# yeyupiaoling/VoiceprintRecognition-PaddlePaddle

Hardware: NVIDIA H100
Metric: utterances/sec ECAPA-TDNN Fbank80 3s embed extract (higher is better)
Workload: dtype bf16x3 (split-bf16 operands, fp32 accumulate; fp32-grade)

## Files before the change

voiceprintrecognition-paddlepaddle_b200/csrc/asp_fused.cu:

```cuda
#include <stdio.h>
#include <string.h>

#include "common.h"
#include "ptx.cuh"

namespace ppv {

constexpr int AF_NT = 64;
constexpr int AF_A_TILE = 128 * 64 * 2;
constexpr int AF_B_TILE = AF_NT * 64 * 2;
constexpr int AF_X_TILE = AF_NT * 128 * 2;
constexpr int AF_STAGES = 2;
constexpr float LOG2E = 1.4426950408889634f;

template <int NSPLIT>
__global__ void __launch_bounds__(384, 1) asp_fused_kernel(const __grid_constant__ AspFusedParams p) {
    constexpr int NP = (NSPLIT == 3) ? 2 : 1;
    extern __shared__ uint8_t smem_raw[];
    const uint32_t smem_base = (smem_u32(smem_raw) + 1023u) & ~1023u;
    uint8_t* smem_gen = smem_raw + (smem_base - smem_u32(smem_raw));
    const int ksteps = p.K / 64;
    const int a_bytes = ksteps * NP * AF_A_TILE;
    const int b_bytes = ksteps * NP * AF_B_TILE;
    const int stage_bytes = b_bytes + 2 * AF_X_TILE;
    const uint32_t a_base = smem_base;
    const uint32_t s_base = smem_base + a_bytes;
    const uint32_t bar_base = s_base + AF_STAGES * stage_bytes;
    const uint32_t a_full = bar_base, a_empty = bar_base + 8;
    auto b_full = [&](int s) { return bar_base + 16u + 8u * s; };
    auto b_empty = [&](int s) { return bar_base + 32u + 8u * s; };

    const int warp = threadIdx.x >> 5, lane = threadIdx.x & 31;
    if (warp == 0 && lane == 0) {
        prefetch_tmap(&p.mapW);
        prefetch_tmap(&p.mapAtt);
        prefetch_tmap(&p.mapX);
    }
    if (warp == 1 && lane == 0) {
        mbar_init(a_full, 1);
        mbar_init(a_empty, 256);
        for (int s = 0; s < AF_STAGES; ++s) {
            mbar_init(b_full(s), 1);
            mbar_init(b_empty(s), 256);
        }
        fence_mbar_init();
    }
    __syncthreads();
    griddep_launch_dependents();
    griddep_wait();

    const int slabs = p.C / 128;
    const int items = slabs * p.B;
    const int ntiles = (p.T + AF_NT - 1) / AF_NT;

    if (warp == 0) {
        int stage = 0;
        uint32_t phase = 0, a_phase = 0;
        int cur_slab = -1;
        for (int item = blockIdx.x; item < items; item += gridDim.x) {
            const int b = item / slabs, slab = item - b * slabs;
            if (slab != cur_slab) {
                mbar_wait(a_empty, a_phase ^ 1u);
                if (lane == 0) {
                    mbar_arrive_expect_tx(a_full, a_bytes);
                    for (int ks = 0; ks < ksteps; ++ks)
                        for (int pl = 0; pl < NP; ++pl)
                            tma_load_3d(a_base + (ks * NP + pl) * AF_A_TILE, &p.mapW, a_full, ks * 64, slab * 128, pl);
                }
                __syncwarp();
                a_phase ^= 1u;
                cur_slab = slab;
            }
            {
                const int nitem = item + gridDim.x;
                if (nitem < items && lane < 2 * ntiles) {
                    const int nb = nitem / slabs, nslab = nitem - nb * slabs;
                    tma_prefetch_l2_3d(&p.mapX, nslab * 128, nb * p.Tp + p.P + (lane >> 1) * AF_NT, lane & 1);
                }
                __syncwarp();
            }
            const int row0 = b * p.Tp + p.P;
            for (int ft = 0; ft < ntiles; ++ft) {
                mbar_wait(b_empty(stage), phase ^ 1u);
                if (lane == 0) {
                    const uint32_t sb = s_base + stage * stage_bytes;
                    mbar_arrive_expect_tx(b_full(stage), stage_bytes);
                    for (int ks = 0; ks < ksteps; ++ks)
                        for (int pl = 0; pl < NP; ++pl)
                            tma_load_3d(sb + (ks * NP + pl) * AF_B_TILE, &p.mapAtt, b_full(stage), ks * 64, row0 + ft * AF_NT, pl);
                    for (int pl = 0; pl < 2; ++pl)
                        tma_load_3d(sb + b_bytes + pl * AF_X_TILE, &p.mapX, b_full(stage), slab * 128, row0 + ft * AF_NT, pl);
                }
                __syncwarp();
                if (++stage == AF_STAGES) {
                    stage = 0;
                    phase ^= 1u;
                }
            }
        }
    } else if (warp >= 4) {
        const int g = (warp - 4) >> 2, t = threadIdx.x & 127, w = t >> 5, l = t & 31;
        const int cl0 = 64 * g + 16 * w + (l >> 2);
        float acc[AF_NT / 2];
#pragma unroll
        for (int i = 0; i < AF_NT / 2; ++i) acc[i] = 0.f;
        int stage = 0;
        uint32_t phase = 0, a_phase = 0;
        int cur_slab = -1;
        for (int item = blockIdx.x; item < items; item += gridDim.x) {
            const int b = item / slabs, slab = item - b * slabs;
            if (slab != cur_slab) {
                mbar_wait(a_full, a_phase);
                a_phase ^= 1u;
                cur_slab = slab;
            }
            const int nitem = item + gridDim.x;
            const bool last_of_slab = (nitem >= items) || (nitem % slabs != slab);
            float gm[2], m[2], S0[2], S1[2], S2[2];
#pragma unroll
            for (int rr = 0; rr < 2; ++rr) {
                const int64_t goff = int64_t(b) * p.gstat.ld + slab * 128 + cl0 + 8 * rr;
                gm[rr] = __bfloat162float(p.gstat.hi()[goff]) + __bfloat162float(p.gstat.lo()[goff]);
                m[rr] = -INFINITY;
                S0[rr] = S1[rr] = S2[rr] = 0.f;
            }
            const int Tb = p.nvalid ? max(1, min(p.T, p.nvalid[b])) : p.T;
            for (int ft = 0; ft < ntiles; ++ft) {
                mbar_wait(b_full(stage), phase);
                const uint32_t sb = s_base + stage * stage_bytes;
                wgmma_fence_acc(acc);
                wgmma_fence();
                for (int ks = 0; ks < ksteps; ++ks) {
                    const uint64_t a_hi = make_sw128_kmajor_desc(a_base + (ks * NP) * AF_A_TILE + g * 64 * 128);
                    const uint64_t b_hi = make_sw128_kmajor_desc(sb + (ks * NP) * AF_B_TILE);
#pragma unroll
                    for (int k = 0; k < 4; ++k) wgmma_bf16<AF_NT>(acc, a_hi + 2 * k, b_hi + 2 * k, (ks > 0 || k > 0) ? 1u : 0u);
                    if (NSPLIT == 3) {
                        const uint64_t a_lo = make_sw128_kmajor_desc(a_base + (ks * NP + 1) * AF_A_TILE + g * 64 * 128);
                        const uint64_t b_lo = make_sw128_kmajor_desc(sb + (ks * NP + 1) * AF_B_TILE);
#pragma unroll
                        for (int k = 0; k < 4; ++k) wgmma_bf16<AF_NT>(acc, a_lo + 2 * k, b_hi + 2 * k, 1u);
#pragma unroll
                        for (int k = 0; k < 4; ++k) wgmma_bf16<AF_NT>(acc, a_hi + 2 * k, b_lo + 2 * k, 1u);
                    }
                }
                wgmma_commit();
                wgmma_wait<0>();
                wgmma_fence_acc(acc);
                if (ft == ntiles - 1 && last_of_slab) mbar_arrive(a_empty);
                const __nv_bfloat16* xs_hi = reinterpret_cast<const __nv_bfloat16*>(smem_gen + (sb - smem_base) + b_bytes);
                const __nv_bfloat16* xs_lo = xs_hi + AF_X_TILE / 2;
                const int f0 = ft * AF_NT;
#pragma unroll
                for (int rr = 0; rr < 2; ++rr) {
                    float cm = -INFINITY;
#pragma unroll
                    for (int i = 0; i < AF_NT / 8; ++i)
#pragma unroll
                        for (int e = 0; e < 2; ++e)
                            if (f0 + 8 * i + 2 * (l & 3) + e < Tb) cm = fmaxf(cm, acc[4 * i + 2 * rr + e]);
                    if (cm > m[rr]) {
                        const float r = exp2f((m[rr] - cm) * LOG2E);
                        S0[rr] *= r;
                        S1[rr] *= r;
                        S2[rr] *= r;
                        m[rr] = cm;
                    }
                    const float ms = m[rr] * LOG2E;
                    const int cl = cl0 + 8 * rr;
#pragma unroll
                    for (int i = 0; i < AF_NT / 8; ++i)
#pragma unroll
                        for (int e = 0; e < 2; ++e) {
                            const int fl = 8 * i + 2 * (l & 3) + e;
                            if (f0 + fl < Tb) {
                                const int o = fl * 128 + cl;
                                const float xv = __bfloat162float(xs_hi[o]) + __bfloat162float(xs_lo[o]);
                                const float ev = exp2f(fmaf(acc[4 * i + 2 * rr + e], LOG2E, -ms));
                                const float d = xv - gm[rr];
                                const float ed = ev * d;
                                S0[rr] += ev;
                                S1[rr] += ed;
                                S2[rr] = fmaf(ed, d, S2[rr]);
                            }
                        }
                }
                mbar_arrive(b_empty(stage));
                if (++stage == AF_STAGES) {
                    stage = 0;
                    phase ^= 1u;
                }
            }
#pragma unroll
            for (int rr = 0; rr < 2; ++rr) {
#pragma unroll
                for (int off = 1; off <= 2; off <<= 1) {
                    const float om = __shfl_xor_sync(0xffffffffu, m[rr], off), o0 = __shfl_xor_sync(0xffffffffu, S0[rr], off),
                                o1 = __shfl_xor_sync(0xffffffffu, S1[rr], off), o2 = __shfl_xor_sync(0xffffffffu, S2[rr], off);
                    const float mm = fmaxf(m[rr], om);
                    const float ra = S0[rr] > 0.f ? exp2f((m[rr] - mm) * LOG2E) : 0.f, rb = o0 > 0.f ? exp2f((om - mm) * LOG2E) : 0.f;
                    S0[rr] = S0[rr] * ra + o0 * rb;
                    S1[rr] = S1[rr] * ra + o1 * rb;
                    S2[rr] = S2[rr] * ra + o2 * rb;
                    m[rr] = mm;
                }
            }
            if ((l & 3) != 0) continue;
            const int C = p.C;
#pragma unroll
            for (int rr = 0; rr < 2; ++rr) {
                const int c = slab * 128 + cl0 + 8 * rr;
                const float inv = 1.f / S0[rr];
                const float dm = S1[rr] * inv;
                const float mean = gm[rr] + dm;
                const float sd = sqrtf(fmaxf(S2[rr] * inv - dm * dm, p.eps));
                if (p.out_raw) {
                    p.out_raw[int64_t(b) * 2 * C + c] = mean;
                    p.out_raw[int64_t(b) * 2 * C + C + c] = sd;
                }
                __nv_bfloat16 h, lo;
                split_bf16(fmaf(mean, p.bn_scale[c], p.bn_shift[c]), h, lo);
                p.out.hi()[int64_t(b) * p.out.ld + c] = h;
                p.out.lo()[int64_t(b) * p.out.ld + c] = lo;
                split_bf16(fmaf(sd, p.bn_scale[C + c], p.bn_shift[C + c]), h, lo);
                p.out.hi()[int64_t(b) * p.out.ld + C + c] = h;
                p.out.lo()[int64_t(b) * p.out.ld + C + c] = lo;
            }
        }
    }
}

int asp_fused_build(AspFusedParams* p, const Planes& W, const Planes& att, const Planes& x, const Planes& gstat, const float* bn_scale,
                    const float* bn_shift, const Planes& out, float* out_raw, int B, int T, int P, int Tp, int C, int K, float eps) {
    PPV_REQUIRE(C % 128 == 0 && K % 64 == 0 && K <= 128, "asp_fused: C % 128 == 0 and K in {64,128} required");
    memset(p, 0, sizeof(*p));
    PPV_REQUIRE(x.ld == C, "asp_fused: x row length must equal C");
    int rc = encode_planes_map(&p->mapW, W, 128);
    if (rc) return rc;
    rc = encode_planes_map(&p->mapAtt, att, AF_NT);
    if (rc) return rc;
    rc = encode_planes_map_ex(&p->mapX, x, 128, AF_NT, 0);
    if (rc) return rc;
    p->x = x;
    p->gstat = gstat;
    p->bn_scale = bn_scale;
    p->bn_shift = bn_shift;
    p->out = out;
    p->out_raw = out_raw;
    p->B = B;
    p->T = T;
    p->P = P;
    p->Tp = Tp;
    p->C = C;
    p->K = K;
    p->eps = eps;
    p->nvalid = nullptr;
    return PPV_OK;
}

int asp_fused_launch(const AspFusedParams& p, int precision, int num_sms, cudaStream_t st) {
    const bool x3 = precision == PPV_PREC_BF16X3;
    const int ksteps = p.K / 64, np = x3 ? 2 : 1;
    const int smem = 1024 + ksteps * np * AF_A_TILE + AF_STAGES * (ksteps * np * AF_B_TILE + 2 * AF_X_TILE) + 96 + 128 * 16 + 64;
    static bool attr3 = false, attr1 = false;
    bool& attr = x3 ? attr3 : attr1;
    if (!attr) {
        if (x3)
            PPV_CUDA_OK(cudaFuncSetAttribute(asp_fused_kernel<3>, cudaFuncAttributeMaxDynamicSharedMemorySize, 227 * 1024));
        else
            PPV_CUDA_OK(cudaFuncSetAttribute(asp_fused_kernel<1>, cudaFuncAttributeMaxDynamicSharedMemorySize, 227 * 1024));
        attr = true;
    }
    const int items = (p.C / 128) * p.B;
    const int grid = std::min(items, num_sms);
    if (x3)
        PPV_PDL_OK(launch_pdl(asp_fused_kernel<3>, dim3(grid), dim3(384), size_t(smem), st, p), "asp_fused_kernel");
    else
        PPV_PDL_OK(launch_pdl(asp_fused_kernel<1>, dim3(grid), dim3(384), size_t(smem), st, p), "asp_fused_kernel");
    return PPV_OK;
}

}
```

voiceprintrecognition-paddlepaddle_b200/csrc/ptx.cuh:

```cuda
#pragma once
#include <cuda.h>
#include <cuda_bf16.h>
#include <cuda_runtime.h>
#include <stdint.h>
#include <stdio.h>

namespace ppv {

__device__ __forceinline__ uint32_t smem_u32(const void* p) {
    return static_cast<uint32_t>(__cvta_generic_to_shared(p));
}

__device__ __forceinline__ bool elect_one() {
    uint32_t pred = 0;
    asm volatile(
        "{\n\t.reg .pred P;\n\t"
        "elect.sync _|P, 0xffffffff;\n\t"
        "selp.u32 %0, 1, 0, P;\n\t}\n"
        : "=r"(pred));
    return pred != 0;
}

__device__ __forceinline__ void mbar_init(uint32_t bar, uint32_t count) {
    asm volatile("mbarrier.init.shared::cta.b64 [%0], %1;" ::"r"(bar), "r"(count) : "memory");
}
__device__ __forceinline__ void fence_mbar_init() {
    asm volatile("fence.mbarrier_init.release.cluster;" ::: "memory");
}
__device__ __forceinline__ void mbar_arrive(uint32_t bar) {
    asm volatile("mbarrier.arrive.shared::cta.b64 _, [%0];" ::"r"(bar) : "memory");
}
__device__ __forceinline__ void mbar_arrive_expect_tx(uint32_t bar, uint32_t bytes) {
    asm volatile("mbarrier.arrive.expect_tx.shared::cta.b64 _, [%0], %1;" ::"r"(bar), "r"(bytes) : "memory");
}
__device__ __forceinline__ uint32_t mbar_try_wait(uint32_t bar, uint32_t parity) {
    uint32_t done;
    asm volatile(
        "{\n\t.reg .pred P;\n\t"
        "mbarrier.try_wait.parity.shared::cta.b64 P, [%1], %2;\n\t"
        "selp.u32 %0, 1, 0, P;\n\t}\n"
        : "=r"(done)
        : "r"(bar), "r"(parity)
        : "memory");
    return done;
}
__device__ __forceinline__ uint64_t global_timer_ns() {
    uint64_t t;
    asm volatile("mov.u64 %0, %%globaltimer;" : "=l"(t));
    return t;
}
__device__ __forceinline__ void mbar_wait(uint32_t bar, uint32_t parity) {
    if (mbar_try_wait(bar, parity)) return;
    const uint64_t t0 = global_timer_ns();
    uint32_t spins = 0;
    while (!mbar_try_wait(bar, parity)) {
        if ((++spins & 0x3ff) == 0 && global_timer_ns() - t0 > 4000000000ull) __trap();
    }
}

template <int N>
__device__ __forceinline__ void setmaxnreg_dec() { asm volatile("setmaxnreg.dec.sync.aligned.u32 %0;" ::"n"(N)); }
template <int N>
__device__ __forceinline__ void setmaxnreg_inc() { asm volatile("setmaxnreg.inc.sync.aligned.u32 %0;" ::"n"(N)); }

__device__ __forceinline__ void prefetch_tmap(const CUtensorMap* m) {
    asm volatile("prefetch.tensormap [%0];" ::"l"(reinterpret_cast<uint64_t>(m)) : "memory");
}
__device__ __forceinline__ void tma_load_3d(uint32_t smem_dst, const CUtensorMap* m, uint32_t bar, int c0, int c1,
                                            int c2) {
    asm volatile(
        "cp.async.bulk.tensor.3d.shared::cluster.global.mbarrier::complete_tx::bytes"
        " [%0], [%1, {%3, %4, %5}], [%2];"
        :
        : "r"(smem_dst), "l"(reinterpret_cast<uint64_t>(m)), "r"(bar), "r"(c0), "r"(c1), "r"(c2)
        : "memory");
}
__device__ __forceinline__ void tma_prefetch_l2_3d(const CUtensorMap* m, int c0, int c1, int c2) {
    asm volatile("cp.async.bulk.prefetch.tensor.3d.L2.global.tile [%0, {%1, %2, %3}];"
                 :
                 : "l"(reinterpret_cast<uint64_t>(m)), "r"(c0), "r"(c1), "r"(c2)
                 : "memory");
}
__device__ __forceinline__ void tma_store_3d(const CUtensorMap* m, uint32_t smem_src, int c0, int c1, int c2) {
    asm volatile("cp.async.bulk.tensor.3d.global.shared::cta.bulk_group [%0, {%2, %3, %4}], [%1];"
                 :
                 : "l"(reinterpret_cast<uint64_t>(m)), "r"(smem_src), "r"(c0), "r"(c1), "r"(c2)
                 : "memory");
}
__device__ __forceinline__ void bulk_commit_group() { asm volatile("cp.async.bulk.commit_group;" ::: "memory"); }
__device__ __forceinline__ void bulk_wait_read0() { asm volatile("cp.async.bulk.wait_group.read 0;" ::: "memory"); }
__device__ __forceinline__ void bulk_wait_all() { asm volatile("cp.async.bulk.wait_group 0;" ::: "memory"); }
__device__ __forceinline__ void fence_proxy_async_smem() { asm volatile("fence.proxy.async.shared::cta;" ::: "memory"); }
__device__ __forceinline__ void bulk_load_1d(uint32_t smem_dst, const void* gsrc, uint32_t bytes, uint32_t bar) {
    asm volatile(
        "cp.async.bulk.shared::cluster.global.mbarrier::complete_tx::bytes [%0], [%1], %2, [%3];"
        :
        : "r"(smem_dst), "l"(reinterpret_cast<uint64_t>(gsrc)), "r"(bytes), "r"(bar)
        : "memory");
}

__device__ __forceinline__ void wgmma_fence() { asm volatile("wgmma.fence.sync.aligned;" ::: "memory"); }
__device__ __forceinline__ void wgmma_commit() { asm volatile("wgmma.commit_group.sync.aligned;" ::: "memory"); }
template <int N>
__device__ __forceinline__ void wgmma_wait() { asm volatile("wgmma.wait_group.sync.aligned %0;" ::"n"(N) : "memory"); }
template <int R>
__device__ __forceinline__ void wgmma_fence_acc(float (&d)[R]) {
#pragma unroll
    for (int i = 0; i < R; ++i) asm volatile("" : "+f"(d[i])::"memory");
}
__device__ __forceinline__ void wgmma_m64n32k16(float (&d)[16], uint64_t desc_a, uint64_t desc_b, uint32_t scale_d) {
    asm volatile(
        "{\n\t.reg .pred p;\n\t"
        "setp.ne.b32 p, %18, 0;\n\t"
        "wgmma.mma_async.sync.aligned.m64n32k16.f32.bf16.bf16 "
        "{%0, %1, %2, %3, %4, %5, %6, %7, %8, %9, %10, %11, %12, %13, %14, %15}, "
        "%16, %17, p, 1, 1, 0, 0;\n\t}\n"
        : "+f"(d[0]), "+f"(d[1]), "+f"(d[2]), "+f"(d[3]), "+f"(d[4]), "+f"(d[5]), "+f"(d[6]), "+f"(d[7]), "+f"(d[8]), "+f"(d[9]), "+f"(d[10]), "+f"(d[11]), "+f"(d[12]), "+f"(d[13]), "+f"(d[14]), "+f"(d[15])
        : "l"(desc_a), "l"(desc_b), "r"(scale_d));
}
__device__ __forceinline__ void wgmma_m64n64k16(float (&d)[32], uint64_t desc_a, uint64_t desc_b, uint32_t scale_d) {
    asm volatile(
        "{\n\t.reg .pred p;\n\t"
        "setp.ne.b32 p, %34, 0;\n\t"
        "wgmma.mma_async.sync.aligned.m64n64k16.f32.bf16.bf16 "
        "{%0, %1, %2, %3, %4, %5, %6, %7, %8, %9, %10, %11, %12, %13, %14, %15, %16, %17, %18, %19, %20, %21, %22, %23, %24, %25, %26, %27, %28, %29, %30, %31}, "
        "%32, %33, p, 1, 1, 0, 0;\n\t}\n"
        : "+f"(d[0]), "+f"(d[1]), "+f"(d[2]), "+f"(d[3]), "+f"(d[4]), "+f"(d[5]), "+f"(d[6]), "+f"(d[7]), "+f"(d[8]), "+f"(d[9]), "+f"(d[10]), "+f"(d[11]), "+f"(d[12]), "+f"(d[13]), "+f"(d[14]), "+f"(d[15]), "+f"(d[16]), "+f"(d[17]), "+f"(d[18]), "+f"(d[19]), "+f"(d[20]), "+f"(d[21]), "+f"(d[22]), "+f"(d[23]), "+f"(d[24]), "+f"(d[25]), "+f"(d[26]), "+f"(d[27]), "+f"(d[28]), "+f"(d[29]), "+f"(d[30]), "+f"(d[31])
        : "l"(desc_a), "l"(desc_b), "r"(scale_d));
}
__device__ __forceinline__ void wgmma_m64n128k16(float (&d)[64], uint64_t desc_a, uint64_t desc_b, uint32_t scale_d) {
    asm volatile(
        "{\n\t.reg .pred p;\n\t"
        "setp.ne.b32 p, %66, 0;\n\t"
        "wgmma.mma_async.sync.aligned.m64n128k16.f32.bf16.bf16 "
        "{%0, %1, %2, %3, %4, %5, %6, %7, %8, %9, %10, %11, %12, %13, %14, %15, %16, %17, %18, %19, %20, %21, %22, %23, %24, %25, %26, %27, %28, %29, %30, %31, %32, %33, %34, %35, %36, %37, %38, %39, %40, %41, %42, %43, %44, %45, %46, %47, %48, %49, %50, %51, %52, %53, %54, %55, %56, %57, %58, %59, %60, %61, %62, %63}, "
        "%64, %65, p, 1, 1, 0, 0;\n\t}\n"
        : "+f"(d[0]), "+f"(d[1]), "+f"(d[2]), "+f"(d[3]), "+f"(d[4]), "+f"(d[5]), "+f"(d[6]), "+f"(d[7]), "+f"(d[8]), "+f"(d[9]), "+f"(d[10]), "+f"(d[11]), "+f"(d[12]), "+f"(d[13]), "+f"(d[14]), "+f"(d[15]), "+f"(d[16]), "+f"(d[17]), "+f"(d[18]), "+f"(d[19]), "+f"(d[20]), "+f"(d[21]), "+f"(d[22]), "+f"(d[23]), "+f"(d[24]), "+f"(d[25]), "+f"(d[26]), "+f"(d[27]), "+f"(d[28]), "+f"(d[29]), "+f"(d[30]), "+f"(d[31]), "+f"(d[32]), "+f"(d[33]), "+f"(d[34]), "+f"(d[35]), "+f"(d[36]), "+f"(d[37]), "+f"(d[38]), "+f"(d[39]), "+f"(d[40]), "+f"(d[41]), "+f"(d[42]), "+f"(d[43]), "+f"(d[44]), "+f"(d[45]), "+f"(d[46]), "+f"(d[47]), "+f"(d[48]), "+f"(d[49]), "+f"(d[50]), "+f"(d[51]), "+f"(d[52]), "+f"(d[53]), "+f"(d[54]), "+f"(d[55]), "+f"(d[56]), "+f"(d[57]), "+f"(d[58]), "+f"(d[59]), "+f"(d[60]), "+f"(d[61]), "+f"(d[62]), "+f"(d[63])
        : "l"(desc_a), "l"(desc_b), "r"(scale_d));
}
__device__ __forceinline__ void wgmma_m64n256k16(float (&d)[128], uint64_t desc_a, uint64_t desc_b, uint32_t scale_d) {
    asm volatile(
        "{\n\t.reg .pred p;\n\t"
        "setp.ne.b32 p, %130, 0;\n\t"
        "wgmma.mma_async.sync.aligned.m64n256k16.f32.bf16.bf16 "
        "{%0, %1, %2, %3, %4, %5, %6, %7, %8, %9, %10, %11, %12, %13, %14, %15, %16, %17, %18, %19, %20, %21, %22, %23, %24, %25, %26, %27, %28, %29, %30, %31, %32, %33, %34, %35, %36, %37, %38, %39, %40, %41, %42, %43, %44, %45, %46, %47, %48, %49, %50, %51, %52, %53, %54, %55, %56, %57, %58, %59, %60, %61, %62, %63, %64, %65, %66, %67, %68, %69, %70, %71, %72, %73, %74, %75, %76, %77, %78, %79, %80, %81, %82, %83, %84, %85, %86, %87, %88, %89, %90, %91, %92, %93, %94, %95, %96, %97, %98, %99, %100, %101, %102, %103, %104, %105, %106, %107, %108, %109, %110, %111, %112, %113, %114, %115, %116, %117, %118, %119, %120, %121, %122, %123, %124, %125, %126, %127}, "
        "%128, %129, p, 1, 1, 0, 0;\n\t}\n"
        : "+f"(d[0]), "+f"(d[1]), "+f"(d[2]), "+f"(d[3]), "+f"(d[4]), "+f"(d[5]), "+f"(d[6]), "+f"(d[7]), "+f"(d[8]), "+f"(d[9]), "+f"(d[10]), "+f"(d[11]), "+f"(d[12]), "+f"(d[13]), "+f"(d[14]), "+f"(d[15]), "+f"(d[16]), "+f"(d[17]), "+f"(d[18]), "+f"(d[19]), "+f"(d[20]), "+f"(d[21]), "+f"(d[22]), "+f"(d[23]), "+f"(d[24]), "+f"(d[25]), "+f"(d[26]), "+f"(d[27]), "+f"(d[28]), "+f"(d[29]), "+f"(d[30]), "+f"(d[31]), "+f"(d[32]), "+f"(d[33]), "+f"(d[34]), "+f"(d[35]), "+f"(d[36]), "+f"(d[37]), "+f"(d[38]), "+f"(d[39]), "+f"(d[40]), "+f"(d[41]), "+f"(d[42]), "+f"(d[43]), "+f"(d[44]), "+f"(d[45]), "+f"(d[46]), "+f"(d[47]), "+f"(d[48]), "+f"(d[49]), "+f"(d[50]), "+f"(d[51]), "+f"(d[52]), "+f"(d[53]), "+f"(d[54]), "+f"(d[55]), "+f"(d[56]), "+f"(d[57]), "+f"(d[58]), "+f"(d[59]), "+f"(d[60]), "+f"(d[61]), "+f"(d[62]), "+f"(d[63]), "+f"(d[64]), "+f"(d[65]), "+f"(d[66]), "+f"(d[67]), "+f"(d[68]), "+f"(d[69]), "+f"(d[70]), "+f"(d[71]), "+f"(d[72]), "+f"(d[73]), "+f"(d[74]), "+f"(d[75]), "+f"(d[76]), "+f"(d[77]), "+f"(d[78]), "+f"(d[79]), "+f"(d[80]), "+f"(d[81]), "+f"(d[82]), "+f"(d[83]), "+f"(d[84]), "+f"(d[85]), "+f"(d[86]), "+f"(d[87]), "+f"(d[88]), "+f"(d[89]), "+f"(d[90]), "+f"(d[91]), "+f"(d[92]), "+f"(d[93]), "+f"(d[94]), "+f"(d[95]), "+f"(d[96]), "+f"(d[97]), "+f"(d[98]), "+f"(d[99]), "+f"(d[100]), "+f"(d[101]), "+f"(d[102]), "+f"(d[103]), "+f"(d[104]), "+f"(d[105]), "+f"(d[106]), "+f"(d[107]), "+f"(d[108]), "+f"(d[109]), "+f"(d[110]), "+f"(d[111]), "+f"(d[112]), "+f"(d[113]), "+f"(d[114]), "+f"(d[115]), "+f"(d[116]), "+f"(d[117]), "+f"(d[118]), "+f"(d[119]), "+f"(d[120]), "+f"(d[121]), "+f"(d[122]), "+f"(d[123]), "+f"(d[124]), "+f"(d[125]), "+f"(d[126]), "+f"(d[127])
        : "l"(desc_a), "l"(desc_b), "r"(scale_d));
}
template <int N>
__device__ __forceinline__ void wgmma_bf16(float (&d)[N / 2], uint64_t desc_a, uint64_t desc_b, uint32_t scale_d) {
    if constexpr (N == 32) wgmma_m64n32k16(d, desc_a, desc_b, scale_d);
    else if constexpr (N == 64) wgmma_m64n64k16(d, desc_a, desc_b, scale_d);
    else if constexpr (N == 128) wgmma_m64n128k16(d, desc_a, desc_b, scale_d);
    else wgmma_m64n256k16(d, desc_a, desc_b, scale_d);
}

__device__ __forceinline__ uint64_t make_sw128_kmajor_desc(uint32_t smem_addr) {
    uint64_t d = 0;
    d |= static_cast<uint64_t>((smem_addr >> 4) & 0x3fff);
    d |= static_cast<uint64_t>(1) << 16;
    d |= static_cast<uint64_t>(1024 >> 4) << 32;
    d |= static_cast<uint64_t>(1) << 62;
    return d;
}
__device__ __forceinline__ uint64_t make_sw64_kmajor_desc(uint32_t smem_addr) {
    uint64_t d = 0;
    d |= static_cast<uint64_t>((smem_addr >> 4) & 0x3fff);
    d |= static_cast<uint64_t>(1) << 16;
    d |= static_cast<uint64_t>(512 >> 4) << 32;
    d |= static_cast<uint64_t>(2) << 62;
    return d;
}

__device__ __forceinline__ void griddep_launch_dependents() { asm volatile("griddepcontrol.launch_dependents;" ::: "memory"); }
__device__ __forceinline__ void griddep_wait() { asm volatile("griddepcontrol.wait;" ::: "memory"); }

__device__ __forceinline__ void named_bar_sync(int id, int nthreads) {
    asm volatile("bar.sync %0, %1;" ::"r"(id), "r"(nthreads) : "memory");
}
__device__ __forceinline__ void named_bar_sync_if(bool pred, int id, int nthreads) {
    asm volatile(
        "{\n\t.reg .pred p;\n\t"
        "setp.ne.b32 p, %2, 0;\n\t"
        "@p bar.sync %0, %1;\n\t}\n" ::"r"(id),
        "r"(nthreads), "r"(uint32_t(pred))
        : "memory");
}
__device__ __forceinline__ void named_bar_arrive_if(bool pred, int id, int nthreads) {
    asm volatile(
        "{\n\t.reg .pred p;\n\t"
        "setp.ne.b32 p, %2, 0;\n\t"
        "@p bar.arrive %0, %1;\n\t}\n" ::"r"(id),
        "r"(nthreads), "r"(uint32_t(pred))
        : "memory");
}
__device__ __forceinline__ float warp_sum(float v) {
#pragma unroll
    for (int o = 16; o > 0; o >>= 1) v += __shfl_xor_sync(0xffffffffu, v, o);
    return v;
}
__device__ __forceinline__ float warp_max(float v) {
#pragma unroll
    for (int o = 16; o > 0; o >>= 1) v = fmaxf(v, __shfl_xor_sync(0xffffffffu, v, o));
    return v;
}
__device__ __forceinline__ __nv_bfloat16 bf16_rn_fast(float x) { return __low2bfloat16(__floats2bfloat162_rn(x, 0.f)); }
__device__ __forceinline__ void split_bf16(float x, __nv_bfloat16& hi, __nv_bfloat16& lo) {
    hi = bf16_rn_fast(x);
    lo = bf16_rn_fast(x - __bfloat162float(hi));
}
__device__ __forceinline__ void split_pack_bf16x2(float a, float b, uint32_t& hi, uint32_t& lo) {
    const __nv_bfloat162 h = __floats2bfloat162_rn(a, b);
    hi = *reinterpret_cast<const uint32_t*>(&h);
    const float ha = __uint_as_float(hi << 16), hb = __uint_as_float(hi & 0xffff0000u);
    const __nv_bfloat162 l = __floats2bfloat162_rn(a - ha, b - hb);
    lo = *reinterpret_cast<const uint32_t*>(&l);
}
__device__ __forceinline__ float2 unpack_bf16x2(uint32_t u) { return make_float2(__uint_as_float(u << 16), __uint_as_float(u & 0xffff0000u)); }
__device__ __forceinline__ uint32_t pack_bf16x2(__nv_bfloat16 a, __nv_bfloat16 b) {
    return static_cast<uint32_t>(__bfloat16_as_ushort(a)) | (static_cast<uint32_t>(__bfloat16_as_ushort(b)) << 16);
}

}
```

Measured before the change: 46930.

## Load X tile with swizzled 64-col TMA boxes and ldmatrix.trans in ASP epilogue

Splits each X tile TMA load into two 64-column boxes using a 128B swizzle, and reads them in the attentive-statistics epilogue with ldmatrix.x4.trans into registers laid out to match the wgmma accumulator fragments. This replaces per-element scalar bf16 shared loads, which likely hit bank conflicts. Because the reads now finish before the math, the stage-empty barrier is released earlier. The masked accumulations become branch-free selects. The cost is more TMA issues per stage, more L2 prefetch calls, and a dependence on the swizzle/lane address math being correct.

```diff
diff --git a/voiceprintrecognition-paddlepaddle_b200/csrc/asp_fused.cu b/voiceprintrecognition-paddlepaddle_b200/csrc/asp_fused.cu
--- a/voiceprintrecognition-paddlepaddle_b200/csrc/asp_fused.cu
+++ b/voiceprintrecognition-paddlepaddle_b200/csrc/asp_fused.cu
@@ -10,6 +10,7 @@
 constexpr int AF_A_TILE = 128 * 64 * 2;
 constexpr int AF_B_TILE = AF_NT * 64 * 2;
 constexpr int AF_X_TILE = AF_NT * 128 * 2;
+constexpr int AF_X_BOX = AF_NT * 64 * 2;
 constexpr int AF_STAGES = 2;
 constexpr float LOG2E = 1.4426950408889634f;
 
@@ -18,7 +19,6 @@
     constexpr int NP = (NSPLIT == 3) ? 2 : 1;
     extern __shared__ uint8_t smem_raw[];
     const uint32_t smem_base = (smem_u32(smem_raw) + 1023u) & ~1023u;
-    uint8_t* smem_gen = smem_raw + (smem_base - smem_u32(smem_raw));
     const int ksteps = p.K / 64;
     const int a_bytes = ksteps * NP * AF_A_TILE;
     const int b_bytes = ksteps * NP * AF_B_TILE;
@@ -73,9 +73,10 @@
             }
             {
                 const int nitem = item + gridDim.x;
-                if (nitem < items && lane < 2 * ntiles) {
+                if (nitem < items) {
                     const int nb = nitem / slabs, nslab = nitem - nb * slabs;
-                    tma_prefetch_l2_3d(&p.mapX, nslab * 128, nb * p.Tp + p.P + (lane >> 1) * AF_NT, lane & 1);
+                    for (int q = lane; q < 4 * ntiles; q += 32)
+                        tma_prefetch_l2_3d(&p.mapX, nslab * 128 + 64 * ((q >> 1) & 1), nb * p.Tp + p.P + (q >> 2) * AF_NT, q & 1);
                 }
                 __syncwarp();
             }
@@ -89,7 +90,9 @@
                         for (int pl = 0; pl < NP; ++pl)
                             tma_load_3d(sb + (ks * NP + pl) * AF_B_TILE, &p.mapAtt, b_full(stage), ks * 64, row0 + ft * AF_NT, pl);
                     for (int pl = 0; pl < 2; ++pl)
-                        tma_load_3d(sb + b_bytes + pl * AF_X_TILE, &p.mapX, b_full(stage), slab * 128, row0 + ft * AF_NT, pl);
+                        for (int h = 0; h < 2; ++h)
+                            tma_load_3d(sb + b_bytes + pl * AF_X_TILE + h * AF_X_BOX, &p.mapX, b_full(stage), slab * 128 + 64 * h,
+                                        row0 + ft * AF_NT, pl);
                 }
                 __syncwarp();
                 if (++stage == AF_STAGES) {
@@ -101,6 +104,8 @@
     } else if (warp >= 4) {
         const int g = (warp - 4) >> 2, t = threadIdx.x & 127, w = t >> 5, l = t & 31;
         const int cl0 = 64 * g + 16 * w + (l >> 2);
+        const int q = l >> 3, r = l & 7;
+        const uint32_t x_lane = uint32_t(g * AF_X_BOX + (8 * (q >> 1) + r) * 128 + (((2 * w + (q & 1)) ^ r) << 4));
         float acc[AF_NT / 2];
 #pragma unroll
         for (int i = 0; i < AF_NT / 2; ++i) acc[i] = 0.f;
@@ -148,8 +153,17 @@
                 wgmma_wait<0>();
                 wgmma_fence_acc(acc);
                 if (ft == ntiles - 1 && last_of_slab) mbar_arrive(a_empty);
-                const __nv_bfloat16* xs_hi = reinterpret_cast<const __nv_bfloat16*>(smem_gen + (sb - smem_base) + b_bytes);
-                const __nv_bfloat16* xs_lo = xs_hi + AF_X_TILE / 2;
+                uint32_t xv[2][AF_NT / 8][2];
+#pragma unroll
+                for (int pl = 0; pl < 2; ++pl)
+#pragma unroll
+                    for (int i2 = 0; i2 < AF_NT / 16; ++i2) {
+                        uint32_t d[4];
+                        ldmatrix_x4_trans(d, sb + b_bytes + pl * AF_X_TILE + i2 * 16 * 128 + x_lane);
+#pragma unroll
+                        for (int qq = 0; qq < 4; ++qq) xv[pl][2 * i2 + (qq >> 1)][qq & 1] = d[qq];
+                    }
+                mbar_arrive(b_empty(stage));
                 const int f0 = ft * AF_NT;
 #pragma unroll
                 for (int rr = 0; rr < 2; ++rr) {
@@ -157,8 +171,7 @@
 #pragma unroll
                     for (int i = 0; i < AF_NT / 8; ++i)
 #pragma unroll
-                        for (int e = 0; e < 2; ++e)
-                            if (f0 + 8 * i + 2 * (l & 3) + e < Tb) cm = fmaxf(cm, acc[4 * i + 2 * rr + e]);
+                        for (int e = 0; e < 2; ++e) cm = f0 + 8 * i + 2 * (l & 3) + e < Tb ? fmaxf(cm, acc[4 * i + 2 * rr + e]) : cm;
                     if (cm > m[rr]) {
                         const float r = exp2f((m[rr] - cm) * LOG2E);
                         S0[rr] *= r;
@@ -167,25 +180,22 @@
                         m[rr] = cm;
                     }
                     const float ms = m[rr] * LOG2E;
-                    const int cl = cl0 + 8 * rr;
-#pragma unroll
-                    for (int i = 0; i < AF_NT / 8; ++i)
+#pragma unroll
+                    for (int i = 0; i < AF_NT / 8; ++i) {
+                        const float2 xh = unpack_bf16x2(xv[0][i][rr]), xl = unpack_bf16x2(xv[1][i][rr]);
 #pragma unroll
                         for (int e = 0; e < 2; ++e) {
-                            const int fl = 8 * i + 2 * (l & 3) + e;
-                            if (f0 + fl < Tb) {
-                                const int o = fl * 128 + cl;
-                                const float xv = __bfloat162float(xs_hi[o]) + __bfloat162float(xs_lo[o]);
-                                const float ev = exp2f(fmaf(acc[4 * i + 2 * rr + e], LOG2E, -ms));
-                                const float d = xv - gm[rr];
-                                const float ed = ev * d;
-                                S0[rr] += ev;
-                                S1[rr] += ed;
-                                S2[rr] = fmaf(ed, d, S2[rr]);
-                            }
+                            const bool valid = f0 + 8 * i + 2 * (l & 3) + e < Tb;
+                            const float x = e ? xh.y + xl.y : xh.x + xl.x;
+                            const float ev = exp2f(fmaf(acc[4 * i + 2 * rr + e], LOG2E, -ms));
+                            const float d = x - gm[rr];
+                            const float ed = ev * d;
+                            S0[rr] = valid ? S0[rr] + ev : S0[rr];
+                            S1[rr] = valid ? S1[rr] + ed : S1[rr];
+                            S2[rr] = valid ? fmaf(ed, d, S2[rr]) : S2[rr];
                         }
-                }
-                mbar_arrive(b_empty(stage));
+                    }
+                }
                 if (++stage == AF_STAGES) {
                     stage = 0;
                     phase ^= 1u;
@@ -239,7 +249,7 @@
     if (rc) return rc;
     rc = encode_planes_map(&p->mapAtt, att, AF_NT);
     if (rc) return rc;
-    rc = encode_planes_map_ex(&p->mapX, x, 128, AF_NT, 0);
+    rc = encode_planes_map_ex(&p->mapX, x, 64, AF_NT, 128);
     if (rc) return rc;
     p->x = x;
     p->gstat = gstat;
diff --git a/voiceprintrecognition-paddlepaddle_b200/csrc/ptx.cuh b/voiceprintrecognition-paddlepaddle_b200/csrc/ptx.cuh
--- a/voiceprintrecognition-paddlepaddle_b200/csrc/ptx.cuh
+++ b/voiceprintrecognition-paddlepaddle_b200/csrc/ptx.cuh
@@ -156,6 +156,13 @@
     else wgmma_m64n256k16(d, desc_a, desc_b, scale_d);
 }
 
+__device__ __forceinline__ void ldmatrix_x4_trans(uint32_t (&d)[4], uint32_t smem_addr) {
+    asm volatile("ldmatrix.sync.aligned.m8n8.x4.trans.shared.b16 {%0, %1, %2, %3}, [%4];"
+                 : "=r"(d[0]), "=r"(d[1]), "=r"(d[2]), "=r"(d[3])
+                 : "r"(smem_addr)
+                 : "memory");
+}
+
 __device__ __forceinline__ uint64_t make_sw128_kmajor_desc(uint32_t smem_addr) {
     uint64_t d = 0;
     d |= static_cast<uint64_t>((smem_addr >> 4) & 0x3fff);
```

Result: no change. 47300, median of 6 (+0.8%).

## Double-buffer wgmma accumulators and split x loads into separate swizzled ring

Applied to the files above, without the earlier changes.

Restructures the fused attentive-statistics-pooling kernel so consumers issue the next tile's wgmma into a second accumulator before running softmax/statistics on the current one. This overlaps tensor-core work with the exp/accumulate epilogue. The attention-operand ring deepens to three stages, and the x tiles move to their own two-stage ring, loaded as 64-column swizzled boxes and read with ldmatrix.trans instead of scalar bf16 shared loads. This costs twice the accumulator registers and more complex barrier and phase bookkeeping.

```diff
diff --git a/voiceprintrecognition-paddlepaddle_b200/csrc/asp_fused.cu b/voiceprintrecognition-paddlepaddle_b200/csrc/asp_fused.cu
--- a/voiceprintrecognition-paddlepaddle_b200/csrc/asp_fused.cu
+++ b/voiceprintrecognition-paddlepaddle_b200/csrc/asp_fused.cu
@@ -9,26 +9,34 @@
 constexpr int AF_NT = 64;
 constexpr int AF_A_TILE = 128 * 64 * 2;
 constexpr int AF_B_TILE = AF_NT * 64 * 2;
-constexpr int AF_X_TILE = AF_NT * 128 * 2;
-constexpr int AF_STAGES = 2;
+constexpr int AF_X_BOX = AF_NT * 64 * 2;
+constexpr int AF_X_STAGE = 2 * 2 * AF_X_BOX;
+constexpr int AF_B_STAGES = 3;
+constexpr int AF_X_STAGES = 2;
+constexpr int AF_BARS = 2 + 2 * AF_B_STAGES + 2 * AF_X_STAGES;
 constexpr float LOG2E = 1.4426950408889634f;
+
+static int asp_fused_smem_bytes(int K, int np) {
+    return 1024 + (K / 64) * np * (AF_A_TILE + AF_B_STAGES * AF_B_TILE) + AF_X_STAGES * AF_X_STAGE + 8 * AF_BARS;
+}
 
 template <int NSPLIT>
 __global__ void __launch_bounds__(384, 1) asp_fused_kernel(const __grid_constant__ AspFusedParams p) {
     constexpr int NP = (NSPLIT == 3) ? 2 : 1;
     extern __shared__ uint8_t smem_raw[];
     const uint32_t smem_base = (smem_u32(smem_raw) + 1023u) & ~1023u;
-    uint8_t* smem_gen = smem_raw + (smem_base - smem_u32(smem_raw));
     const int ksteps = p.K / 64;
     const int a_bytes = ksteps * NP * AF_A_TILE;
     const int b_bytes = ksteps * NP * AF_B_TILE;
-    const int stage_bytes = b_bytes + 2 * AF_X_TILE;
     const uint32_t a_base = smem_base;
-    const uint32_t s_base = smem_base + a_bytes;
-    const uint32_t bar_base = s_base + AF_STAGES * stage_bytes;
+    const uint32_t b_base = a_base + a_bytes;
+    const uint32_t x_base = b_base + AF_B_STAGES * b_bytes;
+    const uint32_t bar_base = x_base + AF_X_STAGES * AF_X_STAGE;
     const uint32_t a_full = bar_base, a_empty = bar_base + 8;
     auto b_full = [&](int s) { return bar_base + 16u + 8u * s; };
-    auto b_empty = [&](int s) { return bar_base + 32u + 8u * s; };
+    auto b_empty = [&](int s) { return bar_base + 16u + 8u * (AF_B_STAGES + s); };
+    auto x_full = [&](int s) { return bar_base + 16u + 8u * (2 * AF_B_STAGES + s); };
+    auto x_empty = [&](int s) { return bar_base + 16u + 8u * (2 * AF_B_STAGES + AF_X_STAGES + s); };
 
     const int warp = threadIdx.x >> 5, lane = threadIdx.x & 31;
     if (warp == 0 && lane == 0) {
@@ -39,9 +47,13 @@
     if (warp == 1 && lane == 0) {
         mbar_init(a_full, 1);
         mbar_init(a_empty, 256);
-        for (int s = 0; s < AF_STAGES; ++s) {
+        for (int s = 0; s < AF_B_STAGES; ++s) {
             mbar_init(b_full(s), 1);
             mbar_init(b_empty(s), 256);
+        }
+        for (int s = 0; s < AF_X_STAGES; ++s) {
+            mbar_init(x_full(s), 1);
+            mbar_init(x_empty(s), 256);
         }
         fence_mbar_init();
     }
@@ -52,145 +64,157 @@
     const int slabs = p.C / 128;
     const int items = slabs * p.B;
     const int ntiles = (p.T + AF_NT - 1) / AF_NT;
+    const int ntot = ((items - 1 - int(blockIdx.x)) / int(gridDim.x) + 1) * ntiles;
+    auto item_of = [&](int j) { return int(blockIdx.x) + (j / ntiles) * int(gridDim.x); };
 
     if (warp == 0) {
-        int stage = 0;
-        uint32_t phase = 0, a_phase = 0;
+        uint32_t a_phase = 0;
         int cur_slab = -1;
-        for (int item = blockIdx.x; item < items; item += gridDim.x) {
-            const int b = item / slabs, slab = item - b * slabs;
-            if (slab != cur_slab) {
-                mbar_wait(a_empty, a_phase ^ 1u);
+        for (int j = 0; j <= ntot; ++j) {
+            if (j < ntot) {
+                const int item = item_of(j), ft = j % ntiles;
+                const int b = item / slabs, slab = item - b * slabs;
+                if (ft == 0 && slab != cur_slab) {
+                    mbar_wait(a_empty, a_phase ^ 1u);
+                    if (lane == 0) {
+                        mbar_arrive_expect_tx(a_full, a_bytes);
+                        for (int ks = 0; ks < ksteps; ++ks)
+                            for (int pl = 0; pl < NP; ++pl)
+                                tma_load_3d(a_base + (ks * NP + pl) * AF_A_TILE, &p.mapW, a_full, ks * 64, slab * 128, pl);
+                    }
+                    __syncwarp();
+                    a_phase ^= 1u;
+                    cur_slab = slab;
+                }
+                const int s = j % AF_B_STAGES;
+                mbar_wait(b_empty(s), ((j / AF_B_STAGES) & 1) ^ 1u);
                 if (lane == 0) {
-                    mbar_arrive_expect_tx(a_full, a_bytes);
+                    const uint32_t sb = b_base + s * b_bytes;
+                    mbar_arrive_expect_tx(b_full(s), b_bytes);
                     for (int ks = 0; ks < ksteps; ++ks)
                         for (int pl = 0; pl < NP; ++pl)
-                            tma_load_3d(a_base + (ks * NP + pl) * AF_A_TILE, &p.mapW, a_full, ks * 64, slab * 128, pl);
+                            tma_load_3d(sb + (ks * NP + pl) * AF_B_TILE, &p.mapAtt, b_full(s), ks * 64, b * p.Tp + p.P + ft * AF_NT, pl);
                 }
                 __syncwarp();
-                a_phase ^= 1u;
-                cur_slab = slab;
-            }
-            {
-                const int nitem = item + gridDim.x;
-                if (nitem < items && lane < 2 * ntiles) {
-                    const int nb = nitem / slabs, nslab = nitem - nb * slabs;
-                    tma_prefetch_l2_3d(&p.mapX, nslab * 128, nb * p.Tp + p.P + (lane >> 1) * AF_NT, lane & 1);
+            }
+            if (j > 0) {
+                const int jx = j - 1;
+                const int item = item_of(jx), ft = jx % ntiles;
+                const int b = item / slabs, slab = item - b * slabs;
+                const int s = jx % AF_X_STAGES;
+                mbar_wait(x_empty(s), ((jx / AF_X_STAGES) & 1) ^ 1u);
+                if (lane == 0) {
+                    const uint32_t sx = x_base + s * AF_X_STAGE;
+                    mbar_arrive_expect_tx(x_full(s), AF_X_STAGE);
+                    for (int pl = 0; pl < 2; ++pl)
+                        for (int h = 0; h < 2; ++h)
+                            tma_load_3d(sx + (pl * 2 + h) * AF_X_BOX, &p.mapX, x_full(s), slab * 128 + h * 64, b * p.Tp + p.P + ft * AF_NT, pl);
                 }
                 __syncwarp();
-            }
-            const int row0 = b * p.Tp + p.P;
-            for (int ft = 0; ft < ntiles; ++ft) {
-                mbar_wait(b_empty(stage), phase ^ 1u);
-                if (lane == 0) {
-                    const uint32_t sb = s_base + stage * stage_bytes;
-                    mbar_arrive_expect_tx(b_full(stage), stage_bytes);
-                    for (int ks = 0; ks < ksteps; ++ks)
-                        for (int pl = 0; pl < NP; ++pl)
-                            tma_load_3d(sb + (ks * NP + pl) * AF_B_TILE, &p.mapAtt, b_full(stage), ks * 64, row0 + ft * AF_NT, pl);
-                    for (int pl = 0; pl < 2; ++pl)
-                        tma_load_3d(sb + b_bytes + pl * AF_X_TILE, &p.mapX, b_full(stage), slab * 128, row0 + ft * AF_NT, pl);
-                }
-                __syncwarp();
-                if (++stage == AF_STAGES) {
-                    stage = 0;
-                    phase ^= 1u;
-                }
             }
         }
     } else if (warp >= 4) {
         const int g = (warp - 4) >> 2, t = threadIdx.x & 127, w = t >> 5, l = t & 31;
         const int cl0 = 64 * g + 16 * w + (l >> 2);
-        float acc[AF_NT / 2];
-#pragma unroll
-        for (int i = 0; i < AF_NT / 2; ++i) acc[i] = 0.f;
-        int stage = 0;
-        uint32_t phase = 0, a_phase = 0;
+        const int r8 = l & 7, mj = l >> 3;
+        const uint32_t x_lane = uint32_t(g * AF_X_BOX + (8 * (mj >> 1) + r8) * 128 + (((2 * w + (mj & 1)) ^ r8) << 4));
+        float accA[AF_NT / 2], accB[AF_NT / 2];
+#pragma unroll
+        for (int i = 0; i < AF_NT / 2; ++i) accA[i] = accB[i] = 0.f;
+        uint32_t a_phase = 0;
         int cur_slab = -1;
-        for (int item = blockIdx.x; item < items; item += gridDim.x) {
-            const int b = item / slabs, slab = item - b * slabs;
+        float gm[2], m[2], S0[2], S1[2], S2[2];
+        int Tb = p.T;
+
+        auto weights_for = [&](int j) {
+            const int slab = item_of(j) % slabs;
             if (slab != cur_slab) {
+                wgmma_wait<0>();
+                if (cur_slab >= 0) mbar_arrive(a_empty);
                 mbar_wait(a_full, a_phase);
                 a_phase ^= 1u;
                 cur_slab = slab;
             }
-            const int nitem = item + gridDim.x;
-            const bool last_of_slab = (nitem >= items) || (nitem % slabs != slab);
-            float gm[2], m[2], S0[2], S1[2], S2[2];
+        };
+        auto issue = [&](float (&acc)[AF_NT / 2], int j) {
+            const int s = j % AF_B_STAGES;
+            mbar_wait(b_full(s), (j / AF_B_STAGES) & 1);
+            const uint32_t sb = b_base + s * b_bytes;
+            wgmma_fence_acc(acc);
+            wgmma_fence();
+            for (int ks = 0; ks < ksteps; ++ks) {
+                const uint64_t a_hi = make_sw128_kmajor_desc(a_base + (ks * NP) * AF_A_TILE + g * 64 * 128);
+                const uint64_t b_hi = make_sw128_kmajor_desc(sb + (ks * NP) * AF_B_TILE);
+#pragma unroll
+                for (int k = 0; k < 4; ++k) wgmma_bf16<AF_NT>(acc, a_hi + 2 * k, b_hi + 2 * k, (ks > 0 || k > 0) ? 1u : 0u);
+                if (NSPLIT == 3) {
+                    const uint64_t a_lo = make_sw128_kmajor_desc(a_base + (ks * NP + 1) * AF_A_TILE + g * 64 * 128);
+                    const uint64_t b_lo = make_sw128_kmajor_desc(sb + (ks * NP + 1) * AF_B_TILE);
+#pragma unroll
+                    for (int k = 0; k < 4; ++k) wgmma_bf16<AF_NT>(acc, a_lo + 2 * k, b_hi + 2 * k, 1u);
+#pragma unroll
+                    for (int k = 0; k < 4; ++k) wgmma_bf16<AF_NT>(acc, a_hi + 2 * k, b_lo + 2 * k, 1u);
+                }
+            }
+            wgmma_commit();
+        };
+        auto softmax = [&](const float (&acc)[AF_NT / 2], int j) {
+            const int item = item_of(j), ft = j % ntiles;
+            const int b = item / slabs, slab = item - b * slabs;
+            if (ft == 0) {
+#pragma unroll
+                for (int rr = 0; rr < 2; ++rr) {
+                    const int64_t goff = int64_t(b) * p.gstat.ld + slab * 128 + cl0 + 8 * rr;
+                    gm[rr] = __bfloat162float(p.gstat.hi()[goff]) + __bfloat162float(p.gstat.lo()[goff]);
+                    m[rr] = -INFINITY;
+                    S0[rr] = S1[rr] = S2[rr] = 0.f;
+                }
+                Tb = p.nvalid ? max(1, min(p.T, p.nvalid[b])) : p.T;
+            }
+            const int s = j % AF_X_STAGES;
+            mbar_wait(x_full(s), (j / AF_X_STAGES) & 1);
+            uint32_t xr[2][4][4];
+#pragma unroll
+            for (int pl = 0; pl < 2; ++pl)
+#pragma unroll
+                for (int n = 0; n < 4; ++n) ldmatrix_x4_trans(xr[pl][n], x_base + s * AF_X_STAGE + pl * 2 * AF_X_BOX + x_lane + n * 16 * 128);
+            mbar_arrive(x_empty(s));
+            const int f0 = ft * AF_NT;
 #pragma unroll
             for (int rr = 0; rr < 2; ++rr) {
-                const int64_t goff = int64_t(b) * p.gstat.ld + slab * 128 + cl0 + 8 * rr;
-                gm[rr] = __bfloat162float(p.gstat.hi()[goff]) + __bfloat162float(p.gstat.lo()[goff]);
-                m[rr] = -INFINITY;
-                S0[rr] = S1[rr] = S2[rr] = 0.f;
-            }
-            const int Tb = p.nvalid ? max(1, min(p.T, p.nvalid[b])) : p.T;
-            for (int ft = 0; ft < ntiles; ++ft) {
-                mbar_wait(b_full(stage), phase);
-                const uint32_t sb = s_base + stage * stage_bytes;
-                wgmma_fence_acc(acc);
-                wgmma_fence();
-                for (int ks = 0; ks < ksteps; ++ks) {
-                    const uint64_t a_hi = make_sw128_kmajor_desc(a_base + (ks * NP) * AF_A_TILE + g * 64 * 128);
-                    const uint64_t b_hi = make_sw128_kmajor_desc(sb + (ks * NP) * AF_B_TILE);
-#pragma unroll
-                    for (int k = 0; k < 4; ++k) wgmma_bf16<AF_NT>(acc, a_hi + 2 * k, b_hi + 2 * k, (ks > 0 || k > 0) ? 1u : 0u);
-                    if (NSPLIT == 3) {
-                        const uint64_t a_lo = make_sw128_kmajor_desc(a_base + (ks * NP + 1) * AF_A_TILE + g * 64 * 128);
-                        const uint64_t b_lo = make_sw128_kmajor_desc(sb + (ks * NP + 1) * AF_B_TILE);
-#pragma unroll
-                        for (int k = 0; k < 4; ++k) wgmma_bf16<AF_NT>(acc, a_lo + 2 * k, b_hi + 2 * k, 1u);
-#pragma unroll
-                        for (int k = 0; k < 4; ++k) wgmma_bf16<AF_NT>(acc, a_hi + 2 * k, b_lo + 2 * k, 1u);
+                float cm = -INFINITY;
+#pragma unroll
+                for (int i = 0; i < AF_NT / 8; ++i)
+#pragma unroll
+                    for (int e = 0; e < 2; ++e)
+                        if (f0 + 8 * i + 2 * (l & 3) + e < Tb) cm = fmaxf(cm, acc[4 * i + 2 * rr + e]);
+                if (cm > m[rr]) {
+                    const float r = exp2f((m[rr] - cm) * LOG2E);
+                    S0[rr] *= r;
+                    S1[rr] *= r;
+                    S2[rr] *= r;
+                    m[rr] = cm;
+                }
+                const float ms = m[rr] * LOG2E;
+#pragma unroll
+                for (int i = 0; i < AF_NT / 8; ++i)
+#pragma unroll
+                    for (int e = 0; e < 2; ++e) {
+                        const int fl = 8 * i + 2 * (l & 3) + e;
+                        if (f0 + fl < Tb) {
+                            const uint32_t xh = xr[0][i >> 1][2 * (i & 1) + rr], xl = xr[1][i >> 1][2 * (i & 1) + rr];
+                            const float xv = (e ? __uint_as_float(xh & 0xffff0000u) : __uint_as_float(xh << 16)) +
+                                             (e ? __uint_as_float(xl & 0xffff0000u) : __uint_as_float(xl << 16));
+                            const float ev = exp2f(fmaf(acc[4 * i + 2 * rr + e], LOG2E, -ms));
+                            const float d = xv - gm[rr];
+                            const float ed = ev * d;
+                            S0[rr] += ev;
+                            S1[rr] += ed;
+                            S2[rr] = fmaf(ed, d, S2[rr]);
+                        }
                     }
-                }
-                wgmma_commit();
-                wgmma_wait<0>();
-                wgmma_fence_acc(acc);
-                if (ft == ntiles - 1 && last_of_slab) mbar_arrive(a_empty);
-                const __nv_bfloat16* xs_hi = reinterpret_cast<const __nv_bfloat16*>(smem_gen + (sb - smem_base) + b_bytes);
-                const __nv_bfloat16* xs_lo = xs_hi + AF_X_TILE / 2;
-                const int f0 = ft * AF_NT;
-#pragma unroll
-                for (int rr = 0; rr < 2; ++rr) {
-                    float cm = -INFINITY;
-#pragma unroll
-                    for (int i = 0; i < AF_NT / 8; ++i)
-#pragma unroll
-                        for (int e = 0; e < 2; ++e)
-                            if (f0 + 8 * i + 2 * (l & 3) + e < Tb) cm = fmaxf(cm, acc[4 * i + 2 * rr + e]);
-                    if (cm > m[rr]) {
-                        const float r = exp2f((m[rr] - cm) * LOG2E);
-                        S0[rr] *= r;
-                        S1[rr] *= r;
-                        S2[rr] *= r;
-                        m[rr] = cm;
-                    }
-                    const float ms = m[rr] * LOG2E;
-                    const int cl = cl0 + 8 * rr;
-#pragma unroll
-                    for (int i = 0; i < AF_NT / 8; ++i)
-#pragma unroll
-                        for (int e = 0; e < 2; ++e) {
-                            const int fl = 8 * i + 2 * (l & 3) + e;
-                            if (f0 + fl < Tb) {
-                                const int o = fl * 128 + cl;
-                                const float xv = __bfloat162float(xs_hi[o]) + __bfloat162float(xs_lo[o]);
-                                const float ev = exp2f(fmaf(acc[4 * i + 2 * rr + e], LOG2E, -ms));
-                                const float d = xv - gm[rr];
-                                const float ed = ev * d;
-                                S0[rr] += ev;
-                                S1[rr] += ed;
-                                S2[rr] = fmaf(ed, d, S2[rr]);
-                            }
-                        }
-                }
-                mbar_arrive(b_empty(stage));
-                if (++stage == AF_STAGES) {
-                    stage = 0;
-                    phase ^= 1u;
-                }
-            }
+            }
+            if (ft != ntiles - 1) return;
 #pragma unroll
             for (int rr = 0; rr < 2; ++rr) {
 #pragma unroll
@@ -205,7 +229,7 @@
                     m[rr] = mm;
                 }
             }
-            if ((l & 3) != 0) continue;
+            if ((l & 3) != 0) return;
             const int C = p.C;
 #pragma unroll
             for (int rr = 0; rr < 2; ++rr) {
@@ -226,6 +250,28 @@
                 p.out.hi()[int64_t(b) * p.out.ld + C + c] = h;
                 p.out.lo()[int64_t(b) * p.out.ld + C + c] = lo;
             }
+        };
+        auto step = [&](float (&cur)[AF_NT / 2], float (&nxt)[AF_NT / 2], int j) {
+            const bool more = j + 1 < ntot;
+            if (more) {
+                weights_for(j + 1);
+                issue(nxt, j + 1);
+                wgmma_wait<1>();
+            } else {
+                wgmma_wait<0>();
+            }
+            wgmma_fence_acc(cur);
+            mbar_arrive(b_empty(j % AF_B_STAGES));
+            softmax(cur, j);
+            return more;
+        };
+        wgmma_fence_acc(accA);
+        wgmma_fence_acc(accB);
+        weights_for(0);
+        issue(accA, 0);
+        for (int j = 0;; j += 2) {
+            if (!step(accA, accB, j)) break;
+            if (!step(accB, accA, j + 1)) break;
         }
     }
 }
@@ -239,7 +285,7 @@
     if (rc) return rc;
     rc = encode_planes_map(&p->mapAtt, att, AF_NT);
     if (rc) return rc;
-    rc = encode_planes_map_ex(&p->mapX, x, 128, AF_NT, 0);
+    rc = encode_planes_map(&p->mapX, x, AF_NT);
     if (rc) return rc;
     p->x = x;
     p->gstat = gstat;
@@ -260,8 +306,7 @@
 
 int asp_fused_launch(const AspFusedParams& p, int precision, int num_sms, cudaStream_t st) {
     const bool x3 = precision == PPV_PREC_BF16X3;
-    const int ksteps = p.K / 64, np = x3 ? 2 : 1;
-    const int smem = 1024 + ksteps * np * AF_A_TILE + AF_STAGES * (ksteps * np * AF_B_TILE + 2 * AF_X_TILE) + 96 + 128 * 16 + 64;
+    const int smem = asp_fused_smem_bytes(p.K, x3 ? 2 : 1);
     static bool attr3 = false, attr1 = false;
     bool& attr = x3 ? attr3 : attr1;
     if (!attr) {
diff --git a/voiceprintrecognition-paddlepaddle_b200/csrc/ptx.cuh b/voiceprintrecognition-paddlepaddle_b200/csrc/ptx.cuh
--- a/voiceprintrecognition-paddlepaddle_b200/csrc/ptx.cuh
+++ b/voiceprintrecognition-paddlepaddle_b200/csrc/ptx.cuh
@@ -173,6 +173,13 @@
     return d;
 }
 
+__device__ __forceinline__ void ldmatrix_x4_trans(uint32_t (&r)[4], uint32_t smem_addr) {
+    asm volatile("ldmatrix.sync.aligned.m8n8.x4.trans.shared.b16 {%0, %1, %2, %3}, [%4];"
+                 : "=r"(r[0]), "=r"(r[1]), "=r"(r[2]), "=r"(r[3])
+                 : "r"(smem_addr)
+                 : "memory");
+}
+
 __device__ __forceinline__ void griddep_launch_dependents() { asm volatile("griddepcontrol.launch_dependents;" ::: "memory"); }
 __device__ __forceinline__ void griddep_wait() { asm volatile("griddepcontrol.wait;" ::: "memory"); }
 
```

Result: no change. 46880 before, 46880 after (median of 6 runs) (-0.0%).
